# driskai/scenario_gym

Measured on AMD Instinct MI355X. Metric: entity-steps/sec (batched rollout), higher is better.
Workload: dtype f64

## Files before the change

### scenario_gym_amd/csrc/h_handle.hip

```cpp
#include "sgym_host.hpp"

using namespace sgh;

thread_local std::string sgh::g_create_err;

int sgh::fail(sg_handle *h, int code, const char *fmt, ...)
{
    char buf[512];
    va_list ap;
    va_start(ap, fmt);
    vsnprintf(buf, sizeof buf, fmt, ap);
    va_end(ap);
    if (h) h->err = buf; else g_create_err = buf;
    return code;
}

int sgh::GrowBuf::ensure(sg_handle *h, size_t bytes, bool *grew)
{
    if (grew) *grew = false;
    if (bytes <= cap) return SG_OK;
    if (ptr) HIP_TRY(h, kind == HOST ? hipHostFree(ptr) : hipFree(ptr));
    ptr = nullptr;
    cap = 0;
    HIP_TRY(h, kind == HOST ? hipHostMalloc(&ptr, bytes, hipHostMallocDefault) : hipMalloc(&ptr, bytes));
// ... 31 lines not shown
    if (cfg->device < 0 || cfg->device >= ndev)
        return fail(nullptr, SG_ERR_INVALID, "sg_create: device %d out of range (%d devices)", cfg->device, ndev);
    hipDeviceProp_t prop;
    if (hipGetDeviceProperties(&prop, cfg->device) != hipSuccess)
        return fail(nullptr, SG_ERR_HIP, "sg_create: hipGetDeviceProperties failed");
    if (strncmp(prop.gcnArchName, "gfx950", 6) != 0)
        return fail(nullptr, SG_ERR_NO_DEVICE, "sg_create: device %d is %s; this library is built for gfx950 only",
                    cfg->device, prop.gcnArchName);
    sg_handle *h = new sg_handle();
    h->cfg = *cfg;
    h->R = cfg->n_scenarios;
    h->E = cfg->n_entities;
    int G = 4;
    while (G < h->E && G < 64) G <<= 1;
    h->G = G;
    h->WV = h->E <= 64 ? 1 : (h->E <= 128 ? 2 : (h->E <= 256 ? 4 : (h->E <= 512 ? 8 : (h->E + 63) / 64)));
    h->wide = h->WV > 8;
    if (h->wide && h->R > 65535) {
        delete h;
        return fail(nullptr, SG_ERR_INVALID, "sg_create: more than 65535 scenarios of more than 512 entities in one handle (n_scenarios=%d)", cfg->n_scenarios);
    }
    h->EP = G * h->WV;
    h->sf = sg_social_force{1.5, 1.0, 1.0, 0.0, 0.5, 1.0, std::cos(200.0 / 2 * M_PI / 180), 1.3, 0.0, 0.0, 2.0, 0.1};
    h->NE = (((size_t)h->R * h->EP + 63) / 64) * 64;
    h->tab_min = env_int("SG_TAB_MIN_STEPS", h->tab_min);
    h->chunk_steps = env_int("SG_CHUNK_STEPS", h->chunk_steps);
    h->overlap = env_int("SG_OVERLAP", h->overlap);
    h->ctl_slice = std::max(1, env_int("SG_CTL_SLICE", h->ctl_slice));
    h->ped_serial = env_int("SG_PED_SERIAL", 0) != 0;
    h->crowd_kernel = env_int("SG_CROWD_KERNEL", 1);
    h->crowd_models = env_int("SG_CROWD_MODELS", 1) != 0;
    h->slice_mode = env_int("SG_SLICE", 1);
    h->queue_mode = env_int("SG_QUEUE", 1);
    h->quiet = env_int("SG_QUIET", 1) != 0;
    h->snap_d2d = env_int("SG_SNAP_D2D", 0);
    int prio_lo = 0, prio_hi = 0;
    if (hipSetDevice(cfg->device) != hipSuccess || hipStreamCreate(&h->stream) != hipSuccess ||
        hipDeviceGetStreamPriorityRange(&prio_lo, &prio_hi) != hipSuccess ||
        hipStreamCreateWithPriority(&h->ctl_stream, hipStreamNonBlocking * 0, env_int("SG_CTL_PRIO", 1) ? prio_hi : prio_lo) != hipSuccess ||
        hipEventCreate(&h->ev0) != hipSuccess || hipEventCreate(&h->ev1) != hipSuccess) {
        delete h;
        return fail(nullptr, SG_ERR_HIP, "sg_create: stream/event creation failed");
    }
    {
        int cus = 0;
        if (hipDeviceGetAttribute(&cus, hipDeviceAttributeMultiprocessorCount, cfg->device) == hipSuccess && cus > 0) h->n_simd = 4 * cus;
        else (void)hipGetLastError();
    }
    *out = h;
    return SG_OK;
}

extern "C" int sg_destroy(sg_handle *h)
{
    if (!h) return SG_OK;
    (void)hipSetDevice(h->cfg.device);
    if (h->stream) (void)hipStreamSynchronize(h->stream);
#ifdef SG_RSS_STATS
    {
        unsigned long long c[8];
        (void)hipMemcpyFromSymbol(c, HIP_SYMBOL(sg::sg_rss_stats), sizeof c);
        fprintf(stderr, "rss stats: flushes %llu groups %llu items %llu passes %llu wave-updates %llu lat-lanes %llu long-lanes %llu\n", c[0], c[1], c[2], c[3], c[4], c[5], c[6]);
    }
#endif
#ifdef SG_PHASE_TIMERS
    if (h->p.phase_cycles) {
        unsigned long long c[16];
// ... 223 lines not shown
```

### scenario_gym_amd/csrc/sgym_collide.hpp

```cpp
#pragma once

namespace sg {

struct TileCentre {
    float fs, fc;
    float fx, fy;
    float mag;
    float reach, thr;
    float nthr;
    int ix, iy;
    bool far_out;
};

__device__ __forceinline__ TileCentre tile_centre(bool present, const double *pose, double bcx, double bcy, float rad_thr,
                                                  float nbr_thr, float cell_inv)
{
    TileCentre C;
    const double x = pose[0], y = pose[1];
    sg_sincos_f32(pose[3], C.fs, C.fc);
    const float bcxf = (float)bcx, bcyf = (float)bcy;
    const float nanf_ = __builtin_nanf("");
    C.fx = present ? (float)x + (bcxf * C.fc - bcyf * C.fs) : nanf_;
    C.fy = present ? (float)y + (bcxf * C.fs + bcyf * C.fc) : nanf_;
    C.mag = __builtin_fabsf(C.fx) + __builtin_fabsf(C.fy);
    C.reach = rad_thr + 1.9073486e-6f * C.mag;
    C.thr = C.reach * C.reach;
    const float nreach = nbr_thr + 1.9073486e-6f * C.mag;
    C.nthr = nreach * nreach;
    const float ax = C.fx * cell_inv, ay = C.fy * cell_inv;
    C.ix = present ? (int)__builtin_floorf(ax) : 0;
    C.iy = present ? (int)__builtin_floorf(ay) : 0;
    C.far_out = present && !(__builtin_fabsf(ax) < 4000.0f && __builtin_fabsf(ay) < 4000.0f);
    return C;
}

template <int G>
__device__ __forceinline__ bool ego_near(const TileCentre &C, bool present, bool is_ego, int ego_lane)
{
    float ex, ey, et;
    if (G == 64) {
        ex = __int_as_float(__builtin_amdgcn_readlane(__float_as_int(C.fx), ego_lane));
        ey = __int_as_float(__builtin_amdgcn_readlane(__float_as_int(C.fy), ego_lane));
        et = __int_as_float(__builtin_amdgcn_readlane(__float_as_int(C.thr), ego_lane));
    } else {
        ex = __shfl(C.fx, ego_lane, 64);
        ey = __shfl(C.fy, ego_lane, 64);
        et = __shfl(C.thr, ego_lane, 64);
    }
    const float dx = C.fx - ex, dy = C.fy - ey;
    const float d2 = __builtin_fmaf(dy, dy, dx * dx);
    return present && !is_ego && d2 <= et;
}

template <int G, int WV, bool PED, bool CROWD = false, bool REFINE = false, typename LDS>
__device__ __forceinline__ void tile_collisions_from(const TileCentre &C, bool present, const double *pose, double velx, double vely,
                                                double dtn ,
                                                double bcx, double bcy, float trig_eps,
                                                bool is_ped_type, int sl, int tile0, LDS &L,
                                                uint64_t (&rows_out)[WV], uint64_t (&mult_rows)[WV],
                                                uint64_t (&nbr_out)[WV], bool &dense , bool *crowd_ok = nullptr,
                                                PhaseTimers *ptp = nullptr, bool hetero = false, float rmax_t = 0.0f)
{
#ifdef SG_PHASE_TIMERS
    PhaseTimers ptm_dummy;
    PhaseTimers &ptm = ptp ? *ptp : ptm_dummy;
#endif
    constexpr int TS = G * WV;
    const int slot = sl - tile0;
    const double x = pose[0], y = pose[1];
    const float fs = C.fs, fc = C.fc, fx = C.fx, fy = C.fy, mag = C.mag, reach = C.reach, thr = C.thr, nthr = C.nthr;
    const int ix = C.ix, iy = C.iy;
    const bool far_out = C.far_out;
    PH(8); tile_sync<WV>(); PH(11);
    L.cx[sl] = fx;
    L.cy[sl] = fy;
    L.cen[sl] = make_float2(fx, fy);
    L.sc[sl] = make_float2(fs, fc);
    reinterpret_cast<unsigned long long *>(L.xtab)[sl] = 0ull;
    reinterpret_cast<unsigned long long *>(L.ytab)[sl] = 0ull;
    bool insane = false;
    if (PED) {
        L.px[sl] = (!CROWD || (present && is_ped_type)) ? x : __builtin_nan("");
        L.py[sl] = y; L.vx[sl] = velx; L.vy[sl] = vely;
        L.isped[sl] = present && is_ped_type;
        const double vmag = sg_norm2(velx, vely) + 0.0000000001;
        const double uox = velx / vmag, uoy = vely / vmag, stp = vmag * dtn;
        L.ox[sl] = uox;
        L.oy[sl] = uoy;
        L.stp[sl] = stp;
        if (CROWD) {
            const double sx = stp * uox, sy = stp * uoy;
            L.sx[sl] = sx;
            L.sy[sl] = sy;
            L.ss[sl] = stp * stp;
// ... 205 lines not shown
                    const int j = tile0 + w * 64 + jl;
                    const float2 oc = L.cen[j], os = L.sc[j], oh = L.half[j];
                    float dx = oc.x - fx, dy = oc.y - fy;
                    float cd = __builtin_fabsf(__builtin_fmaf(fc, os.y, fs * os.x));
                    float sd = __builtin_fabsf(__builtin_fmaf(fs, os.y, -(fc * os.x)));
                    float g0 = __builtin_fabsf(__builtin_fmaf(dx, fc, dy * fs)) - __builtin_fmaf(oh.y, sd, __builtin_fmaf(oh.x, cd, hl));
                    float g1 = __builtin_fabsf(__builtin_fmaf(dy, fc, -(dx * fs))) - __builtin_fmaf(oh.y, cd, __builtin_fmaf(oh.x, sd, hw));
                    float g2 = __builtin_fabsf(__builtin_fmaf(dx, os.y, dy * os.x)) - __builtin_fmaf(hw, sd, __builtin_fmaf(hl, cd, oh.x));
                    float g3 = __builtin_fabsf(__builtin_fmaf(dy, os.y, -(dx * os.x))) - __builtin_fmaf(hw, cd, __builtin_fmaf(hl, sd, oh.y));
                    float gap = __builtin_fmaxf(__builtin_fmaxf(g0, g1), __builtin_fmaxf(g2, g3));
                    float eps = __builtin_fmaf(1.9073486e-6f, __builtin_fabsf(oc.x) + __builtin_fabsf(oc.y), eps_own);
                    bool unsure = (gap <= eps) && (gap >= -eps);
                    unsure = unsure || (dx == 0.0f && dy == 0.0f);
                    if (unsure) fuzzy[w] |= 1ull << jl;
                    else if (gap < -eps) rows_out[w] |= 1ull << jl;
                }
            }
            any_fuzzy = any_fuzzy || fuzzy[w] != 0;
        }
    }
#pragma unroll
    for (int w = 0; w < WV; ++w) mult_rows[w] = rows_out[w];
    PH(3);
    const bool any_fuzzy_wg = block_vote<WV>(L, 1, any_fuzzy) != 0;
    PH(15);
    if (!any_fuzzy_wg) return;

    double A[8];
    {
        double s, c;
        const double *Kp = SG_TRIG;
        asm volatile("" : "+s"(Kp));
        sg_sincos(pose[3], s, c, (ConstTbl)Kp);
        sg_corners(x, y, s, c, L.boxwl[0][sl], L.boxwl[1][sl], bcx, bcy, A);
    }
    if (WV > 1) {
#pragma unroll
        for (int k = 0; k < 8; ++k) L.cor[k][sl] = A[k];
        tile_sync<WV>();
    }
    uint64_t eq[WV];
    bool any_eq = false;
#pragma unroll
    for (int w = 0; w < WV; ++w) {
        eq[w] = 0;
        while (sg_any(fuzzy[w] != 0)) {
            const bool act = fuzzy[w] != 0;
            const int jl = act ? __builtin_ctzll(fuzzy[w]) : (slot & 63);
            if (act) fuzzy[w] &= fuzzy[w] - 1;
            const int j = tile0 + w * 64 + jl;
            double B[8];
            bool same = true;
#pragma unroll
            for (int k = 0; k < 8; ++k) {
                B[k] = WV > 1 ? L.cor[k][j] : shfl_d(A[k], j);
                same = same && (B[k] == A[k]);
            }
            if (act) {
                if (same) eq[w] |= 1ull << jl;
                else if (sg_quads_intersect(A, B)) rows_out[w] |= 1ull << jl;
            }
        }
        any_eq = any_eq || eq[w] != 0;
        mult_rows[w] = rows_out[w];
    }
    if (block_vote<WV>(L, 2, any_eq)) {
// ... 41 lines not shown
```

### scenario_gym_amd/csrc/sgym_host.hpp

```cpp
#pragma once
#include <hip/hip_runtime.h>

#include <algorithm>
#include <functional>
#include <atomic>
#include <cassert>
#include <cmath>
#include <cstdarg>
#include <cstdio>
#include <cstdlib>
#include <chrono>
#include <cstring>
#include <iterator>
#include <memory>
#include <string>
#include <thread>
#include <vector>

#include "sgym_launch.hpp"

using sg::Params;

namespace sgh {

// ... 7 lines not shown
struct GrowBuf {
    enum Kind { DEVICE, DEVICE_POISONED, HOST };
    explicit GrowBuf(Kind k) : kind(k) {}
    void *ptr = nullptr;
    size_t cap = 0;
    const Kind kind;
    int ensure(sg_handle *h, size_t bytes, bool *grew = nullptr);
    void release();
    template <typename T> T *as() const { return static_cast<T *>(ptr); }
};

struct EntityList {
    GrowBuf buf{GrowBuf::DEVICE};
    int64_t n = 0;
    int32_t *scenarios() const { return buf.as<int32_t>(); }
    int32_t *slots() const { return buf.as<int32_t>() + buf.cap / (2 * sizeof(int32_t)); }
    int upload(sg_handle *h, int64_t n_new, const int32_t *scenario, const int32_t *slot);
    void release() { buf.release(); }
};

}

struct sg_handle {
    sg_config cfg{};
    int R = 0, E = 0, EP = 0, G = 0, WV = 1;
    size_t NE = 0;
    bool wide = false;
    hipStream_t stream = nullptr;
    hipStream_t ctl_stream = nullptr;
    hipEvent_t ev0 = nullptr, ev1 = nullptr;
    int n_simd = 1024;
    int tab_min = 16, chunk_steps = 1024, overlap = 1;
    int slice_mode = 1;
    bool quiet = true;
    int queue_mode = 1;
    int ctl_slice = 64;
    int ped_serial = 0;
    int crowd_kernel = 1;
    bool crowd_models = true, models_all_sf = true;
    double c_tol = 0.4;
    uint64_t generation = 0, tick_gen = ~0ull;
    std::string err;

    bool uploaded = false;
    bool has_ped = false;
    bool planar = false;
    bool sliceable = false;
    bool all_ped = false;
    bool crowd_riders = false;
    bool ego_first = true;
    Params p{};
    sgh::ReusePool static_allocs, state_allocs;
    int32_t *d_row_scen = nullptr;
    int64_t total_rows = 0;
    std::vector<hipEvent_t> up_ev;
    std::vector<double> up_grid_t;
    sgh::GrowBuf up_stat{sgh::GrowBuf::HOST};
    std::vector<int32_t> up_row_scen;
    std::vector<std::vector<double>> up_grids;
    int n_ctl = 0;
    int n_ext = 0;
    double *d_ext = nullptr;
    int max_ctl_per_block = 0;
    std::vector<double> clock_t0;
    std::vector<int> clock_of;
    std::vector<uint8_t> slot_empty;
    unsigned char *d_reset_mask = nullptr;
// ... 389 lines not shown
```

### scenario_gym_amd/csrc/sgym_rollout.hpp

```cpp
#pragma once

namespace sg {

enum : unsigned {
    V_PED = 1,
    V_TAB = 2,
    V_HAST = 4,
    V_ROAD = 8,
    V_RSS = 16,
    V_CROWD = 32,
    V_SLICE = 64,
    V_PLANAR = 128,
    V_RIDERS = 256,
    V_CTAB = 512,
    V_MODELS = 1024
};

template <int G, int WV, unsigned F>
struct Variant {
    static constexpr bool PED = (F & V_PED) != 0, TAB = (F & V_TAB) != 0, HAST = (F & V_HAST) != 0, ROAD = (F & V_ROAD) != 0,
                          RSSV = (F & V_RSS) != 0, CROWD = (F & V_CROWD) != 0, SLICE = (F & V_SLICE) != 0, PLANAR = (F & V_PLANAR) != 0,
                          RIDERS = (F & V_RIDERS) != 0, CTAB = (F & V_CTAB) != 0, MODELS = !CROWD || (F & V_MODELS) != 0;
    static_assert(F < 2 * V_MODELS, "flags: V_* bits only");
    static_assert(!SLICE || (TAB && WV == 1 && !PED && !ROAD && !RSSV), "slices: the table variant, one wavefront per tile");
// ... 16 lines not shown
                                            const LanePtr &st)
{
    Table T;
    if (kind == SG_KIND_REPLAY) {
        size_t go = (size_t)ss.grid_off;
        T.x = p.grid_t + go; T.xs = 1;
        T.y = p.grid_y + go * 6 * p.EP + slot; T.ys = 6 * p.EP; T.cs = p.EP;
        T.n = ss.grid_n;
    } else if (kind >= SG_KIND_AGENT_REPLAY) {
        const double *kn = p.knots + fld<int64_t>(st, ST_KNOT_OFF) * 7;
        T.x = kn; T.xs = 7; T.y = kn + 1; T.ys = 7; T.cs = 1;
        T.n = (int)(fld<int64_t>(st, ST_META) >> 32);
    } else {
        T.x = nullptr; T.y = nullptr; T.n = 0; T.xs = T.ys = T.cs = 0;
    }
    return T;
}

struct SliceArgs {
    int mode;
    int n_slices, len;
    int n_total;
    const double *tt;
    const int *clock_of;
    double *dnorm;
    double2 *espeed;
    int *first_done;
    sg_event *ev;
    int *nev;
    const int *n_final;
    int slice0;
};

template <int G, int WV, unsigned F>
__device__ __forceinline__ void rollout_body_l(
    typename Variant<G, WV, F>::Lds &lds ,
    const Params &p, double timestep, int n_steps, int do_reset, int force, const double *actions ,
    const double *tab , const SliceArgs &sa = SliceArgs{},
    const unsigned bx_arg = ~0u )
{
    const unsigned bx = bx_arg == ~0u ? blockIdx.x : bx_arg;
    using V = Variant<G, WV, F>;
    constexpr bool PED = V::PED, TAB = V::TAB, ROAD = V::ROAD, RSSV = V::RSSV, CROWD = V::CROWD, SLICE = V::SLICE, PLANAR = V::PLANAR,
                   RIDERS = V::RIDERS, CTAB = V::CTAB, MODELS = V::MODELS;
    constexpr bool HAS_TAB = V::HAS_TAB, REFINE = V::REFINE, LATE = V::LATE, PARK = V::PARK;
    constexpr int NS = V::NS, TL = V::TL;
    const int tid = threadIdx.x, lane = tid & 63, wave = tid >> 6;
    const uint32_t voff = lane * 8u;
    const size_t blk = (size_t)bx * WV + wave;
    const double *st_blk = p.stat + blk * (ST_COUNT * 64);
    const LanePtr st(st_blk, voff);
    const LanePtr dy(p.dyn + blk * ((size_t)(SG_F_COLL + WV) * 64), voff);
    const int gl = bx * NS + tid;
    const int r_raw = WV == 1 ? gl / G : bx;
    const int slot = WV == 1 ? (gl & (G - 1)) : tid;
    const int tile0 = WV == 1 ? (lane & ~(G - 1)) : 0;
    const int sl = tid;
    const bool in_range = r_raw < p.R;
    const uint32_t r = in_range ? r_raw : p.R - 1;
    const ScenStatic &ss = p.sstat[r];
    sg_scenario_state &sd = p.sdyn[r];
    const int64_t meta = fld<int64_t>(st, ST_META);
    const int kind = (in_range && slot < p.E) ? (int)(meta & 0xff) : SG_KIND_NONE;
    const bool is_ped_type = ((meta >> 8) & 0xff) == 1;
    const bool is_ego = in_range && slot == ss.ego;
    const double bcx = fld(st, ST_BCX), bcy = fld(st, ST_BCY);
    const double min_t = fld(st, ST_MIN_T), max_t = fld(st, ST_MAX_T);
    const double length = ss.length;
    const bool is_static = (int)(meta >> 32) == 1;
    const bool is_agent = kind >= SG_KIND_AGENT_REPLAY;
    const bool is_replay = kind == SG_KIND_REPLAY;
    const bool replay_always = p.persist || is_static;
    float rad_thr, trig_eps, nbr_thr = 0.0f;
    float rmax_tile = 0.0f;
    bool hetero = false;
    {
        const double bw = fld(st, ST_BW), bl = fld(st, ST_BL);
        float rad = (float)(0.5 * __builtin_sqrt(bl * bl + bw * bw)) * 1.000001f;
        float off = (float)__builtin_sqrt(bcx * bcx + bcy * bcy) * 1.000001f;
        float rmax = rad, omax = off, omax_ped = (PED && is_ped_type) ? off : 0.0f;
#pragma unroll
        for (int o = 1; o < G; o <<= 1) {
            rmax = __builtin_fmaxf(rmax, __shfl_xor(rmax, o, 64));
            omax = __builtin_fmaxf(omax, __shfl_xor(omax, o, 64));
            if (PED) omax_ped = __builtin_fmaxf(omax_ped, __shfl_xor(omax_ped, o, 64));
        }
        if (WV > 1) {
            float *red = reinterpret_cast<float *>(lds.cor);
            if (lane == 0) { red[wave] = rmax; red[8 + wave] = omax; red[16 + wave] = omax_ped; }
            __syncthreads();
            for (int w = 0; w < WV; ++w) {
                rmax = __builtin_fmaxf(rmax, red[w]); omax = __builtin_fmaxf(omax, red[8 + w]);
                omax_ped = __builtin_fmaxf(omax_ped, red[16 + w]);
            }
            __syncthreads();
        }
        rad_thr = rad + rmax + 2e-3f + 2.0f * SG_TRIG32_ERR * (off + omax);
        trig_eps = SG_TRIG32_ERR * (12.0f * rad_thr + 4.0f * (off + omax));
        if (REFINE) {
// ... 41 lines not shown
                }
            }
            if (tid == 0) { lds.road_info[0] = n_staged; lds.road_info[1] = net; lds.road_info[2] = (int)net_flags; }
        }
    }
    bool crowd_static_ok = false, crowd_geom_ok = false;
    CrowdConsts CC{};
    if (CROWD) {
        const double rr = fld(st, ST_CTRL + SG_C_PED_RADIUS), hr = fld(st, ST_CTRL + SG_C_PED_HEAD_ROT);
        crowd_geom_ok = sg_all(kind != SG_KIND_AGENT_PEDESTRIAN || (hr == 0.0 && rr > 0.0 && rr < 0x1p20)) && !p.ped_serial;
        crowd_static_ok = crowd_geom_ok && crowd_params_ok(p.sf);
        const RecipDiv rs(p.sf.ped_repulse_sigma);
        CC.k2_scale = p.sf.ped_repulse_V / p.sf.ped_repulse_sigma;
        CC.sig_b = rs.b;
        CC.sig_r = rs.r;
        CC.cos_sight = p.sf.cos_sight;
        CC.sight_weight = p.sf.sight_weight;
        CC.k3 = 2 * p.sf.ped_attract_C;
    }
    bool crowd_ok = false;
    float cell_inv;
    {
        float tmax = __builtin_fmaxf(rad_thr, nbr_thr);
#pragma unroll
        for (int o = 1; o < G; o <<= 1) tmax = __builtin_fmaxf(tmax, __shfl_xor(tmax, o, 64));
        if (WV > 1) {
            float *red = reinterpret_cast<float *>(lds.cor);
            if (lane == 0) red[wave] = tmax;
            __syncthreads();
            for (int w = 0; w < WV; ++w) tmax = __builtin_fmaxf(tmax, red[w]);
            __syncthreads();
        }
        cell_inv = 1.0f / (1.05f * tmax + 0.05f);
    }
    const double *wp = nullptr;
    int nwp = 0;
    if (PED && kind == SG_KIND_AGENT_PEDESTRIAN) {
        int64_t rt = fld<int64_t>(st, ST_ROUTE);
        wp = p.routes + (rt & 0xffffffffffffll) * 2;
        nwp = (int)(rt >> 48);
    }

    double pose[6], dist, t, prev_t;
    double velx = 0.0, vely = 0.0;
    CtrlState cs;
    double m_avg, m_max, m_t;
    uint64_t last_row[WV];
    long long noise_pos = 0;
    int n_ev, goal_idx = 0;
    bool present;
    int done, steps;
    uint64_t row[WV], mult_rows[WV], nbr[WV];
    bool dense = false;
    const int64_t ctl_q = HAS_TAB ? fld<int64_t>(st, ST_CTL) : -1;
    const bool tab_lane = HAS_TAB && ctl_q >= 0 && (kind == SG_KIND_AGENT_PID || kind == SG_KIND_AGENT_VEHICLE);
    const size_t tab_lane_stride = (size_t)(p.tab_steps + 1) * CT_W;
    const bool rider = (RIDERS && kind != SG_KIND_NONE && kind != SG_KIND_AGENT_PEDESTRIAN) ||
                       (CTAB && (kind == SG_KIND_AGENT_PID || kind == SG_KIND_AGENT_VEHICLE));
    const double *rider_row = (RIDERS || CTAB) ? tab + (size_t)(rider ? fld<int64_t>(st, ST_CTL) : 0) * tab_lane_stride : nullptr;
    int last_k = -1;
    int cl[TL];
    const double *cb[TL];
    double sx[TL], sy[TL], sh[TL];
    if (HAS_TAB) {
        uint64_t cm = __ballot(tab_lane);
#pragma unroll
// ... 265 lines not shown
        Table T = lane_table(p, kind, ss, slot, st);
        S.cur = seg_locate(T, t);
        seg_load(T, S);
    }

    if (HAS_TAB && n_steps > 0) tab_issue(true);

    int k = 0;
    bool all_done = false;
    bool vel_clean_prev = false;
    const bool vel_every_step = !LATE || (p.term_mask & ~SG_TERM_MAX_LENGTH) != 0 || sg_any(is_ego && !tab_lane);
    auto rows_again = [](const LanePtr &o) {
        LanePtr q = o;
        if (LATE) {
            asm volatile("" : "+v"(q.a[0]));
            q.a[1] = q.a[0] + 8 * ROW;
            q.a[2] = q.a[0] + 16 * ROW;
        }
        return q;
    };
    auto dy_again = [&]() {
        if (!LATE) return dy;
        uint32_t voff_o = voff;
        asm volatile("" : "+v"(voff_o));
        return LanePtr(p.dyn + blk * ((size_t)(SG_F_COLL + WV) * 64), voff_o);
    };
    auto sd_again = [&]() -> sg_scenario_state & {
        if (!LATE) return sd;
        uint32_t r_o = r;
        asm volatile("" : "+v"(r_o));
        return p.sdyn[r_o];
    };
    const bool quiet_on = V::QUIET && p.quiet != 0 && (p.term_mask & ~SG_TERM_MAX_LENGTH) == 0 && p.rec_cap == 0;
    PhaseTimers ptm;
#ifdef SG_PHASE_TIMERS
    ptm.start();
    if (lane == 0 && bx < 1024) p.phase_cycles[16 + bx * 4 + wave] = __builtin_amdgcn_s_getreg((4 << 0) | (0 << 6) | (31 << 11));
#endif
    sg_loads_done();
    sg_lgkm_done();
    while (k < n_steps && !all_done) {
    if (!CROWD && t + timestep > S.x_hi) {
        int kind_o = kind, slot_o = slot;
        LanePtr st_o = st;
        asm volatile("" : "+v"(kind_o), "+v"(slot_o), "+v"(st_o.a[0]));
        Table T = lane_table(p, kind_o, ss, slot_o, st_o);
        seg_advance(T, S, t + timestep);
        sg_loads_done();
    }
    for (; k < n_steps; ++k) {
        if (!CROWD && sg_any(t + timestep > S.x_hi)) break;
        const bool warm = SLICE && k == 0;
        const bool run_lane = in_range && (force || !done) && !(SLICE && k == 0 && slice_a == 0);
        PH(5);
        const bool any_run_ = WV == 1 ? sg_any(run_lane || (SLICE && k == 0 && in_range && !done)) : run_lane;
        PH(7);
        if (!any_run_) { all_done = true; break; }
        const bool run = (G == 64 && WV == 1 && !SLICE) ? true : run_lane;
        const double *Kp = SG_TRIG;
        if (!TAB) asm volatile("" : "+s"(Kp));
        ConstTbl K = (ConstTbl)Kp;

        const double next_t = t + timestep;
        const double state_dt = t - prev_t;
        const double dt = next_t - t;
        double act_a = 0.0, act_s = 0.0;
// ... 218 lines not shown
            RecipDiv rd(dt);
            if (PLANAR) {
                flat = !SLICE && sg_all(dt > 0.0);
            } else {
                const uint32_t zbits = (uint32_t)(__double2hiint(d[2]) | __double2hiint(d[4]) | __double2hiint(d[5])) |
                                       (uint32_t)(__double2loint(d[2]) | __double2loint(d[4]) | __double2loint(d[5]));
                flat = !SLICE && sg_all((!run | !npres | (present & (zbits == 0))) & (dt > 0.0));
            }
            auto lo_ok = [](double a) { return (__builtin_fabs(a) >= 0x1p-959) | (__double_as_longlong(a) == 0); };
            double dmax = __builtin_fmax(__builtin_fmax(__builtin_fabs(d[0]), __builtin_fabs(d[1])), __builtin_fabs(d[3]));
            bool safe = rd.ok & lo_ok(d[0]) & lo_ok(d[1]) & lo_ok(d[3]);
            if (!flat) {
                dmax = __builtin_fmax(__builtin_fmax(dmax, __builtin_fabs(d[2])), __builtin_fmax(__builtin_fabs(d[4]), __builtin_fabs(d[5])));
                safe = safe & lo_ok(d[2]) & lo_ok(d[4]) & lo_ok(d[5]);
            }
            safe = safe & (dmax < 0x1p961);
            if (sg_all(safe)) {
                vel[0] = rd.div(d[0]); vel[1] = rd.div(d[1]); vel[3] = rd.div(d[3]);
                if (flat) {
                    vel[2] = vel[4] = vel[5] = 0.0;
                } else {
                    vel[2] = rd.div(d[2]); vel[4] = rd.div(d[4]); vel[5] = rd.div(d[5]);
                }
            } else {
#pragma unroll
                for (int c = 0; c < 6; ++c) vel[c] = d[c] / dt;
            }
        }

        const bool vel_zpr_clean = vel_clean_prev;
        vel_clean_prev = flat;
        const bool was_present = present;
        if (run) {
            present = npres;
            if (npres) {
                if (PLANAR) {
                    pose[0] = np_[0]; pose[1] = np_[1]; pose[3] = np_[3];
                } else {
#pragma unroll
                    for (int c = 0; c < 6; ++c) pose[c] = np_[c];
                }
                if (!SLICE) dist += PLANAR ? sg_norm2(d[0], d[1])  : sg_norm3(d[0], d[1], d[2]);
                if (PED) { velx = vel[0]; vely = vel[1]; }
            }
            prev_t = t;
            t = next_t;
            ++steps;
            last_k = k;
            if (SLICE && sa.mode == 0 && !warm) {
                sa.dnorm[((size_t)blk * (size_t)(sa.n_total + 1) + (size_t)steps) * 64 + lane] = npres ? sg_norm3(d[0], d[1], d[2]) : 0.0;
                if (is_ego)
                    sa.espeed[(size_t)steps * p.R + r] =
                        make_double2(present ? sg_norm3(vel[0], vel[1], vel[2]) : __builtin_nan(""),
                                     (was_present && steps > 1) ? 1.0 - prev_t / t : __builtin_nan(""));
            }
            if (LATE) {
                if (need_vel && present) {
                    const LanePtr dv = dy_again();
#pragma unroll
                    for (int c = 0; c < 6; ++c) stf(dv, SG_F_VEL + c, vel[c]);
                }
            } else if (!SLICE || (sa.mode == 1 && !warm)) {
            stf(dy, SG_F_POSE + 0, pose[0]); stf(dy, SG_F_POSE + 1, pose[1]); stf(dy, SG_F_POSE + 3, pose[3]);
            if (!flat) { stf(dy, SG_F_POSE + 2, pose[2]); stf(dy, SG_F_POSE + 4, pose[4]); stf(dy, SG_F_POSE + 5, pose[5]); }
            if (present) {
                stf(dy, SG_F_VEL + 0, vel[0]); stf(dy, SG_F_VEL + 1, vel[1]); stf(dy, SG_F_VEL + 3, vel[3]);
                if (!(flat && vel_zpr_clean)) {
                    stf(dy, SG_F_VEL + 2, vel[2]); stf(dy, SG_F_VEL + 4, vel[4]); stf(dy, SG_F_VEL + 5, vel[5]);
                }
            }
            stf(dy, SG_F_DIST, dist);
            if (SLICE || sg_any(present != was_present)) stf(dy, SG_F_PRESENT, (uint64_t)present);
            }
            if (PED && kind == SG_KIND_AGENT_PEDESTRIAN) {
                stf(dy, SG_F_FORCE + 0, fpx);
                stf(dy, SG_F_FORCE + 1, fpy);
            }
            if (p.rec_cap > 0 && steps < p.rec_cap) {
                int nan_hi = 0x7ff80000;
                if (!CROWD) asm volatile("" : "+s"(nan_hi));
                const double absent = __hiloint2double(nan_hi, 0);
#pragma unroll
                for (int c = 0; c < 6; ++c)
                    p.rec_pose[((size_t)steps * 6 + c) * p.R * p.EP + (size_t)r * p.EP + slot] = present ? pose[c] : absent;
                if (slot == 0) { p.rec_t[(size_t)steps * p.R + r] = t; sd_again().rec_rows = steps + 1; }
            }
            if (!SLICE && is_ego && present && !tab_lane) {
                if (CROWD) { m_avg = lds.ego_m[0]; m_max = lds.ego_m[1]; m_t = lds.ego_m[2]; }
                if (PARK) ego_fetch();
                double speed = sg_norm3(vel[0], vel[1], vel[2]);
                double w = m_t / t;
                m_avg += (1.0 - w) * (speed - m_avg);
                m_t = t;
                m_max = __builtin_fmax(speed, m_max);
                if (CROWD) { lds.ego_m[0] = m_avg; lds.ego_m[1] = m_max; lds.ego_m[2] = m_t; }
                if (PARK) ego_park();
            }
        }
        PH(1);
        const TileCentre cen = tile_centre(present, pose, bcx, bcy, rad_thr, nbr_thr, cell_inv);
        bool quiet = false;
        if (V::QUIET && quiet_on && k != n_steps - 1) {
            const bool ends = (p.term_mask & SG_TERM_MAX_LENGTH) && (t + dt > length);
            const uint64_t ego_mask = __ballot(is_ego);
            int ego_lane = (int)__builtin_ctzll(ego_mask | (1ull << 63));
            if (G < 64) {
                const uint32_t half = lane < 32 ? (uint32_t)ego_mask : (uint32_t)(ego_mask >> 32);
                ego_lane = tile0 + (int)(__builtin_ctz((half >> (tile0 & 31)) | 0x80000000u) & (G - 1));
            }
            quiet = !sg_any(run_lane & (ends | ego_near<G>(cen, present, is_ego, ego_lane)));
        }
        if (V::QUIET && quiet) {
            if (run && is_ego) row[0] = 0;
        } else {
            uint64_t nrow[WV];
            tile_collisions_from<G, WV, PED, CROWD, REFINE>(cen, present, pose, velx, vely, (t + timestep) - t, bcx, bcy, trig_eps,
                                                            is_ped_type, sl, tile0, lds, nrow, mult_rows, nbr, dense, &crowd_ok, &ptm, hetero, rmax_tile);
            if (run) {
#pragma unroll
                for (int w = 0; w < WV; ++w) {
                    const bool row_moved = !LATE && (SLICE || sg_any(nrow[w] != row[w]));
                    row[w] = nrow[w];
                    if ((!SLICE || (sa.mode == 1 && !warm)) && row_moved) stf(dy, SG_F_COLL + w, row[w]);
                }
            }
        }

        int ndone = 0;
        if ((p.term_mask & SG_TERM_MAX_LENGTH) && (t + dt > length)) ndone = 1;
        if (p.term_mask & (SG_TERM_COLLISION | SG_TERM_EGO_COLLISION)) {
            bool any_mine = false;
#pragma unroll
            for (int w = 0; w < WV; ++w) any_mine = any_mine || row[w] != 0;
            bool any_tile, ego0;
            if (WV == 1) {
                uint64_t m = __ballot(any_mine) >> tile0;
                if (G < 64) m &= (1ull << (G & 63)) - 1;
                any_tile = m != 0;
                uint64_t row0 = __shfl(row[0], tile0, 64);
                ego0 = ((__ballot(present) >> tile0) & 1) && row0 != 0;
            } else {
                any_tile = __syncthreads_or(any_mine);
                ego0 = __syncthreads_or(tid == 0 && present && any_mine);
            }
            if ((p.term_mask & SG_TERM_COLLISION) && any_tile) ndone = 1;
            if ((p.term_mask & SG_TERM_EGO_COLLISION) && ego0) ndone = 1;
        }
        if (ROAD && (p.term_mask & SG_TERM_EGO_OFF_ROAD)) {
            bool off = false;
            if (sl == tile0 && in_range) {
// ... 147 lines not shown
        } else if ((RIDERS || CTAB) && rider) {
            if (last_k >= 0 && (kind == SG_KIND_AGENT_PID || kind == SG_KIND_AGENT_VEHICLE)) {
                const double *lr = rider_row + (size_t)last_k * CT_W;
                const double *lr1 = lr + (size_t)p.n_ctl_pad * tab_lane_stride;
                stf(dx, SG_F_CTRL + 0, lr[CT_SPEED]); stf(dx, SG_F_CTRL + 1, lr1[CT_ELON]);
                stf(dx, SG_F_CTRL + 2, lr1[CT_ELAT]); stf(dx, SG_F_CTRL + 3, lr1[CT_EINT]);
            }
        } else {
            stf(dx, SG_F_CTRL + 0, cs.speed); stf(dx, SG_F_CTRL + 1, cs.e_lon_prev);
            stf(dx, SG_F_CTRL + 2, cs.e_lat_prev); stf(dx, SG_F_CTRL + 3, cs.e_lon_int);
        }
        if (slot == 0) { sx.t = t; sx.prev_t = prev_t; sx.done = done; sx.n_steps = steps; if (PED) sx.noise_pos = noise_pos; }
        if (RSSV) {
            if (slot < p.E) {
                p.rss_state[rss_idx] = rss_st;
                if (rss_touched) {
                    p.rss_code[rss_idx] = rss_cd;
                    p.rss_safe[(size_t)rss_idx * 2] = rss_lat;
                    p.rss_safe[(size_t)rss_idx * 2 + 1] = rss_long;
                }
            }
            if (slot == 0 && rss_touched) p.rss_seen[r] = steps;
        }
        if (is_ego) {
            sx.ego_avg_speed = m_avg; sx.ego_max_speed = m_max; sx.avg_t = m_t;
            if (steps > 0 && present) sx.ego_distance_travelled = dist;
#pragma unroll
            for (int w = 0; w < WV; ++w) (w < 4 ? sx.last_row[w & 3] : sx.last_row_hi[w & 3]) = last_row[w];
            sx.n_events = n_ev;
        }
    }
}

template <int G, int WV, unsigned F>
__device__ __forceinline__ void rollout_body(
    const Params &p, double timestep, int n_steps, int do_reset, int force, const double *actions, const double *tab,
    const SliceArgs &sa = SliceArgs{}, const unsigned bx_arg = ~0u)
{
    __shared__ typename Variant<G, WV, F>::Lds lds;
    rollout_body_l<G, WV, F>(lds, p, timestep, n_steps, do_reset, force, actions, tab, sa, bx_arg);
}

struct TabGroups {
    unsigned long long active, bufof[2];
    int gsz, n[4];
    const double *buf[4];
    unsigned start0, len0, start1, len1;
    __device__ __forceinline__ unsigned map(unsigned i) const { return i < len0 ? start0 + i : start1 + (i - len0); }
    __device__ __forceinline__ bool pick(unsigned blk, int &n_steps, const double *&tab) const
    {
        const unsigned g = blk / (unsigned)gsz;
        if (!((active >> g) & 1)) return false;
        const unsigned b = (unsigned)(bufof[g >> 5] >> (2 * (g & 31))) & 3u;
        n_steps = b == 0 ? n[0] : (b == 1 ? n[1] : (b == 2 ? n[2] : n[3]));
        tab = b == 0 ? buf[0] : (b == 1 ? buf[1] : (b == 2 ? buf[2] : buf[3]));
        return true;
    }
};

template <int G, int WV, bool PED, bool TAB>
__global__ __launch_bounds__(64 * WV, PED ? SG_WAVES_PER_SIMD_PED : (TAB ? SG_WAVES_PER_SIMD_TAB : SG_WAVES_PER_SIMD)) void rollout_kernel(
    Params p, double timestep, int n_steps, int do_reset, int force, const double *actions, const double *tab)
{
    constexpr unsigned F = (PED ? V_PED : 0u) | (TAB ? V_TAB : 0u) | (TAB && WV > 1 ? V_HAST : 0u);
    rollout_body<G, WV, F>(p, timestep, n_steps, do_reset, force, actions, tab);
}

template <int WV>
__global__ __launch_bounds__(64 * WV, SG_WAVES_PER_SIMD_PED) void rollout_kernel_crowd(
    Params p, double timestep, int n_steps, int do_reset, int force, const double *actions, const double *tab)
{
    rollout_body<64, WV, V_PED | V_CROWD>(p, timestep, n_steps, do_reset, force, actions, tab);
}
// ... 32 lines not shown
{
    int n_steps;
    const double *tab;
    const unsigned blk = tg.map(blockIdx.x);
    if (!tg.pick(blk, n_steps, tab)) return;
    rollout_body<G, 1, V_RSS | V_CTAB>(p, timestep, n_steps, 0, force, nullptr, tab, SliceArgs{}, blk);
}

template <int G, int WV>
__global__ __launch_bounds__(64 * WV, SG_WAVES_PER_SIMD) void rollout_kernel_rss_road(
    Params p, double timestep, int n_steps, int do_reset, int force, const double *actions, const double *tab)
{
    rollout_body<G, WV, V_ROAD | V_RSS>(p, timestep, n_steps, do_reset, force, actions, tab);
}
template <int G, int WV>
__global__ __launch_bounds__(64 * WV, SG_WAVES_PER_SIMD_PED) void rollout_kernel_rss_ped(
    Params p, double timestep, int n_steps, int do_reset, int force, const double *actions, const double *tab)
{
    rollout_body<G, WV, V_PED | V_RSS>(p, timestep, n_steps, do_reset, force, actions, tab);
}

#ifndef SG_TAB_WAVES
#define SG_TAB_WAVES 3
#define SG_TAB_VGPR 84
#endif
template <int G>
__global__ __launch_bounds__(64, SG_TAB_WAVES) __attribute__((amdgpu_num_vgpr(SG_TAB_VGPR))) void rollout_kernel_tab(
    Params p, double timestep, int force, TabGroups tg)
{
    int n_steps;
    const double *tab;
    const unsigned blk = tg.map(blockIdx.x);
    if (!tg.pick(blk, n_steps, tab)) return;
    rollout_body<G, 1, V_TAB | V_HAST>(p, timestep, n_steps, 0, force, nullptr, tab, SliceArgs{}, blk);
}
#ifndef SG_PLANAR_WAVES
#define SG_PLANAR_WAVES 3
#define SG_PLANAR_VGPR 84
#endif
template <int G>
__global__ __launch_bounds__(64, SG_PLANAR_WAVES) __attribute__((amdgpu_num_vgpr(SG_PLANAR_VGPR))) void rollout_kernel_tab_planar(
    Params p, double timestep, int force, TabGroups tg)
{
    int n_steps;
    const double *tab;
    const unsigned blk = tg.map(blockIdx.x);
    if (!tg.pick(blk, n_steps, tab)) return;
    rollout_body<G, 1, V_TAB | V_HAST | V_PLANAR>(p, timestep, n_steps, 0, force, nullptr, tab, SliceArgs{}, blk);
}

template <int G>
__global__ __launch_bounds__(64, SG_WAVES_PER_SIMD_TAB) void rollout_kernel_slice(Params p, double timestep, SliceArgs sa)
{
    rollout_body<G, 1, V_TAB | V_SLICE>(p, timestep, 0, 0, 0, nullptr, nullptr, sa);
}
template <int G>
__global__ __launch_bounds__(64, SG_WAVES_PER_SIMD_TAB) void rollout_kernel_slice_tab(Params p, double timestep, SliceArgs sa, const double *tab)
{
    rollout_body<G, 1, V_TAB | V_HAST | V_SLICE>(p, timestep, 0, 0, 0, nullptr, tab, sa);
}

#ifdef SG_UNIT_MAIN
static __global__ __launch_bounds__(64) void clock_kernel(const double *t0 , int n_clocks, double timestep, int n_total, double *tt)
{
    const int c = blockIdx.x * 64 + threadIdx.x;
    if (c >= n_clocks) return;
    double *row = tt + (size_t)c * (size_t)(n_total + 1);
    double t = t0[c];
    row[0] = t;
    int j = 1;
    for (; j + 15 <= n_total; j += 16) {
        double v[16];
#pragma unroll
        for (int u = 0; u < 16; ++u) { t = t + timestep; v[u] = t; }
#pragma unroll
        for (int u = 0; u < 16; ++u) row[j + u] = v[u];
    }
    for (; j <= n_total; ++j) { t = t + timestep; row[j] = t; }
}
#endif

// ... 127 lines not shown
```

Baseline: 148.8 billion.

## Add conservative ego-distance slack to skip quiet-step proximity checks

```diff
diff --git a/scenario_gym_amd/csrc/h_handle.hip b/scenario_gym_amd/csrc/h_handle.hip
--- a/scenario_gym_amd/csrc/h_handle.hip
+++ b/scenario_gym_amd/csrc/h_handle.hip
@@ -87,7 +87,7 @@
     h->crowd_models = env_int("SG_CROWD_MODELS", 1) != 0;
     h->slice_mode = env_int("SG_SLICE", 1);
     h->queue_mode = env_int("SG_QUEUE", 1);
-    h->quiet = env_int("SG_QUIET", 1) != 0;
+    { const int q = env_int("SG_QUIET", 1); h->quiet = q == 0 ? 0 : q == 2 ? 2 : 1; }
     h->snap_d2d = env_int("SG_SNAP_D2D", 0);
     int prio_lo = 0, prio_hi = 0;
     if (hipSetDevice(cfg->device) != hipSuccess || hipStreamCreate(&h->stream) != hipSuccess ||
diff --git a/scenario_gym_amd/csrc/sgym_collide.hpp b/scenario_gym_amd/csrc/sgym_collide.hpp
--- a/scenario_gym_amd/csrc/sgym_collide.hpp
+++ b/scenario_gym_amd/csrc/sgym_collide.hpp
@@ -12,13 +12,12 @@
     bool far_out;
 };
 
-__device__ __forceinline__ TileCentre tile_centre(bool present, const double *pose, double bcx, double bcy, float rad_thr,
+__device__ __forceinline__ TileCentre tile_centre(bool present, const double *pose, float bcxf, float bcyf, float rad_thr,
                                                   float nbr_thr, float cell_inv)
 {
     TileCentre C;
     const double x = pose[0], y = pose[1];
     sg_sincos_f32(pose[3], C.fs, C.fc);
-    const float bcxf = (float)bcx, bcyf = (float)bcy;
     const float nanf_ = __builtin_nanf("");
     C.fx = present ? (float)x + (bcxf * C.fc - bcyf * C.fs) : nanf_;
     C.fy = present ? (float)y + (bcxf * C.fs + bcyf * C.fc) : nanf_;
@@ -33,9 +32,14 @@
     C.far_out = present && !(__builtin_fabsf(ax) < 4000.0f && __builtin_fabsf(ay) < 4000.0f);
     return C;
 }
+__device__ __forceinline__ TileCentre tile_centre(bool present, const double *pose, double bcx, double bcy, float rad_thr,
+                                                  float nbr_thr, float cell_inv)
+{
+    return tile_centre(present, pose, (float)bcx, (float)bcy, rad_thr, nbr_thr, cell_inv);
+}
 
 template <int G>
-__device__ __forceinline__ bool ego_near(const TileCentre &C, bool present, bool is_ego, int ego_lane)
+__device__ __forceinline__ bool ego_near(const TileCentre &C, bool present, bool is_ego, int ego_lane, float *d2_out = nullptr)
 {
     float ex, ey, et;
     if (G == 64) {
@@ -49,7 +53,56 @@
     }
     const float dx = C.fx - ex, dy = C.fy - ey;
     const float d2 = __builtin_fmaf(dy, dy, dx * dx);
+    if (d2_out) *d2_out = d2;
     return present && !is_ego && d2 <= et;
+}
+
+#define SG_SLACK_EPS 1.0e-5f
+#define SG_SLACK_DELTA 0x1p-15f
+#define SG_SLACK_CAP 256.0f
+#define SG_SLACK_MAG 65536.0f
+
+template <int G>
+__device__ __forceinline__ float ego_bcast(float v, int ego_lane)
+{
+    if (G == 64) return __int_as_float(__builtin_amdgcn_readlane(__float_as_int(v), ego_lane));
+    return __shfl(v, ego_lane, 64);
+}
+
+__device__ __forceinline__ float ego_turn(float bcxf, float bcyf)
+{
+    return (__builtin_fabsf(bcxf) + __builtin_fabsf(bcyf)) * 1.000001f;
+}
+
+__device__ __forceinline__ float ego_move(double step_len, double dh, float bcxf, float bcyf)
+{
+    const float dhf = __builtin_fabsf((float)dh);
+    return __builtin_fmaf(__builtin_fabsf(bcxf), dhf, __builtin_fmaf(__builtin_fabsf(bcyf), dhf, (float)step_len));
+}
+
+template <int G>
+__device__ __forceinline__ float ego_slack_step(float slack, float mv, bool appears, int lane, int ego_lane)
+{
+    const float mv_ego = ego_bcast<G>(mv, ego_lane);
+    slack = __builtin_fmaf(-(1.0f + SG_SLACK_EPS), (mv + mv_ego) + SG_SLACK_DELTA, slack);
+    const uint64_t app = __ballot(appears);
+    if (app) {
+        const uint64_t mine = (1ull << lane) | (1ull << ego_lane);
+        if (app & mine) slack = 0.0f;
+    }
+    return slack;
+}
+
+template <int G>
+__device__ __forceinline__ float ego_slack_refresh(const TileCentre &C, float d2, float off, bool present, int ego_lane)
+{
+    const float er = ego_bcast<G>(C.reach, ego_lane), em = ego_bcast<G>(C.mag, ego_lane), eo = ego_bcast<G>(off, ego_lane);
+    const float D = __builtin_sqrtf(d2);
+    const float margin = __builtin_fmaf(0x1p-19f, D + er, __builtin_fmaf(3.6e-7f, C.mag + em, 4.0e-5f * (off + eo)));
+    const float s = (D - er) - margin;
+    const bool small = (C.mag < SG_SLACK_MAG) & (em < SG_SLACK_MAG);
+    const float kept = small ? (s < SG_SLACK_CAP ? s : SG_SLACK_CAP) : 0.0f;
+    return (!present | (em != em)) ? SG_SLACK_CAP : kept;
 }
 
 template <int G, int WV, bool PED, bool CROWD = false, bool REFINE = false, typename LDS>
@@ -59,7 +112,8 @@
                                                 bool is_ped_type, int sl, int tile0, LDS &L,
                                                 uint64_t (&rows_out)[WV], uint64_t (&mult_rows)[WV],
                                                 uint64_t (&nbr_out)[WV], bool &dense , bool *crowd_ok = nullptr,
-                                                PhaseTimers *ptp = nullptr, bool hetero = false, float rmax_t = 0.0f)
+                                                PhaseTimers *ptp = nullptr, bool hetero = false, float rmax_t = 0.0f,
+                                                const LanePtr *bc_row = nullptr )
 {
 #ifdef SG_PHASE_TIMERS
     PhaseTimers ptm_dummy;
@@ -331,6 +385,11 @@
         const double *Kp = SG_TRIG;
         asm volatile("" : "+s"(Kp));
         sg_sincos(pose[3], s, c, (ConstTbl)Kp);
+        if (bc_row) {
+            bcx = fld(*bc_row, ST_BCX);
+            bcy = fld(*bc_row, ST_BCY);
+            sg_loads_done();
+        }
         sg_corners(x, y, s, c, L.boxwl[0][sl], L.boxwl[1][sl], bcx, bcy, A);
     }
     if (WV > 1) {
diff --git a/scenario_gym_amd/csrc/sgym_host.hpp b/scenario_gym_amd/csrc/sgym_host.hpp
--- a/scenario_gym_amd/csrc/sgym_host.hpp
+++ b/scenario_gym_amd/csrc/sgym_host.hpp
@@ -63,7 +63,7 @@
     int n_simd = 1024;
     int tab_min = 16, chunk_steps = 1024, overlap = 1;
     int slice_mode = 1;
-    bool quiet = true;
+    int quiet = 1;
     int queue_mode = 1;
     int ctl_slice = 64;
     int ped_serial = 0;
diff --git a/scenario_gym_amd/csrc/sgym_rollout.hpp b/scenario_gym_amd/csrc/sgym_rollout.hpp
--- a/scenario_gym_amd/csrc/sgym_rollout.hpp
+++ b/scenario_gym_amd/csrc/sgym_rollout.hpp
@@ -72,7 +72,7 @@
     int slice0;
 };
 
-template <int G, int WV, unsigned F>
+template <int G, int WV, unsigned F, bool SLACK = true>
 __device__ __forceinline__ void rollout_body_l(
     typename Variant<G, WV, F>::Lds &lds ,
     const Params &p, double timestep, int n_steps, int do_reset, int force, const double *actions ,
@@ -105,6 +105,7 @@
     const bool is_ped_type = ((meta >> 8) & 0xff) == 1;
     const bool is_ego = in_range && slot == ss.ego;
     const double bcx = fld(st, ST_BCX), bcy = fld(st, ST_BCY);
+    const float bcxf = (float)bcx, bcyf = (float)bcy;
     const double min_t = fld(st, ST_MIN_T), max_t = fld(st, ST_MAX_T);
     const double length = ss.length;
     const bool is_static = (int)(meta >> 32) == 1;
@@ -212,6 +213,7 @@
             __syncthreads();
         }
         cell_inv = 1.0f / (1.05f * tmax + 0.05f);
+        if (V::QUIET && G == 64) cell_inv = __int_as_float(__builtin_amdgcn_readfirstlane(__float_as_int(cell_inv)));
     }
     const double *wp = nullptr;
     int nwp = 0;
@@ -543,6 +545,17 @@
         return p.sdyn[r_o];
     };
     const bool quiet_on = V::QUIET && p.quiet != 0 && (p.term_mask & ~SG_TERM_MAX_LENGTH) == 0 && p.rec_cap == 0;
+    const bool slack_on = SLACK && quiet_on && p.quiet == 2;
+    float slack = 0.0f;
+    auto ego_lane_of = [&]() {
+        const uint64_t ego_mask = __ballot(is_ego);
+        int ego_lane = (int)__builtin_ctzll(ego_mask | (1ull << 63));
+        if (G < 64) {
+            const uint32_t half = lane < 32 ? (uint32_t)ego_mask : (uint32_t)(ego_mask >> 32);
+            ego_lane = tile0 + (int)(__builtin_ctz((half >> (tile0 & 31)) | 0x80000000u) & (G - 1));
+        }
+        return ego_lane;
+    };
     PhaseTimers ptm;
 #ifdef SG_PHASE_TIMERS
     ptm.start();
@@ -827,6 +840,7 @@
         vel_clean_prev = flat;
         const bool was_present = present;
         if (run) {
+            float mv = 0.0f;
             present = npres;
             if (npres) {
                 if (PLANAR) {
@@ -835,9 +849,14 @@
 #pragma unroll
                     for (int c = 0; c < 6; ++c) pose[c] = np_[c];
                 }
-                if (!SLICE) dist += PLANAR ? sg_norm2(d[0], d[1])  : sg_norm3(d[0], d[1], d[2]);
+                if (!SLICE) {
+                    const double step_len = PLANAR ? sg_norm2(d[0], d[1])  : sg_norm3(d[0], d[1], d[2]);
+                    dist += step_len;
+                    if (V::QUIET && slack_on) mv = ego_move(step_len, d[3], bcxf, bcyf);
+                }
                 if (PED) { velx = vel[0]; vely = vel[1]; }
             }
+            if (V::QUIET && slack_on) slack = ego_slack_step<G>(slack, mv, present & !was_present, lane, ego_lane_of());
             prev_t = t;
             t = next_t;
             ++steps;
@@ -893,24 +912,33 @@
             }
         }
         PH(1);
-        const TileCentre cen = tile_centre(present, pose, bcx, bcy, rad_thr, nbr_thr, cell_inv);
+        const bool eligible = V::QUIET && quiet_on && k != n_steps - 1;
         bool quiet = false;
-        if (V::QUIET && quiet_on && k != n_steps - 1) {
-            const bool ends = (p.term_mask & SG_TERM_MAX_LENGTH) && (t + dt > length);
-            const uint64_t ego_mask = __ballot(is_ego);
-            int ego_lane = (int)__builtin_ctzll(ego_mask | (1ull << 63));
-            if (G < 64) {
-                const uint32_t half = lane < 32 ? (uint32_t)ego_mask : (uint32_t)(ego_mask >> 32);
-                ego_lane = tile0 + (int)(__builtin_ctz((half >> (tile0 & 31)) | 0x80000000u) & (G - 1));
-            }
-            quiet = !sg_any(run_lane & (ends | ego_near<G>(cen, present, is_ego, ego_lane)));
+        bool ends = false;
+        if (V::QUIET && eligible) {
+            ends = (p.term_mask & SG_TERM_MAX_LENGTH) && (t + dt > length);
+            if (slack_on) quiet = !sg_any(run_lane & (ends | (present & !is_ego & !(slack > 0.0f))));
+        }
+        TileCentre cen;
+        if (!(V::QUIET && quiet)) {
+            cen = V::QUIET ? tile_centre(present, pose, bcxf, bcyf, rad_thr, nbr_thr, cell_inv)
+                           : tile_centre(present, pose, bcx, bcy, rad_thr, nbr_thr, cell_inv);
+            if (V::QUIET && eligible) {
+                const int ego_lane = ego_lane_of();
+                float d2;
+                quiet = !sg_any(run_lane & (ends | ego_near<G>(cen, present, is_ego, ego_lane, &d2)));
+                if (slack_on) slack = ego_slack_refresh<G>(cen, d2, ego_turn(bcxf, bcyf), present, ego_lane);
+            }
         }
         if (V::QUIET && quiet) {
             if (run && is_ego) row[0] = 0;
         } else {
             uint64_t nrow[WV];
-            tile_collisions_from<G, WV, PED, CROWD, REFINE>(cen, present, pose, velx, vely, (t + timestep) - t, bcx, bcy, trig_eps,
-                                                            is_ped_type, sl, tile0, lds, nrow, mult_rows, nbr, dense, &crowd_ok, &ptm, hetero, rmax_tile);
+            LanePtr st_o = st;
+            if (V::QUIET) asm volatile("" : "+v"(st_o.a[0]));
+            tile_collisions_from<G, WV, PED, CROWD, REFINE>(cen, present, pose, velx, vely, (t + timestep) - t, V::QUIET ? 0.0 : bcx,
+                                                            V::QUIET ? 0.0 : bcy, trig_eps, is_ped_type, sl, tile0, lds, nrow, mult_rows, nbr,
+                                                            dense, &crowd_ok, &ptm, hetero, rmax_tile, V::QUIET ? &st_o : nullptr);
             if (run) {
 #pragma unroll
                 for (int w = 0; w < WV; ++w) {
@@ -1124,13 +1152,13 @@
     }
 }
 
-template <int G, int WV, unsigned F>
+template <int G, int WV, unsigned F, bool SLACK = true>
 __device__ __forceinline__ void rollout_body(
     const Params &p, double timestep, int n_steps, int do_reset, int force, const double *actions, const double *tab,
     const SliceArgs &sa = SliceArgs{}, const unsigned bx_arg = ~0u)
 {
     __shared__ typename Variant<G, WV, F>::Lds lds;
-    rollout_body_l<G, WV, F>(lds, p, timestep, n_steps, do_reset, force, actions, tab, sa, bx_arg);
+    rollout_body_l<G, WV, F, SLACK>(lds, p, timestep, n_steps, do_reset, force, actions, tab, sa, bx_arg);
 }
 
 struct TabGroups {
@@ -1229,7 +1257,7 @@
     const double *tab;
     const unsigned blk = tg.map(blockIdx.x);
     if (!tg.pick(blk, n_steps, tab)) return;
-    rollout_body<G, 1, V_TAB | V_HAST>(p, timestep, n_steps, 0, force, nullptr, tab, SliceArgs{}, blk);
+    rollout_body<G, 1, V_TAB | V_HAST, false>(p, timestep, n_steps, 0, force, nullptr, tab, SliceArgs{}, blk);
 }
 #ifndef SG_PLANAR_WAVES
 #define SG_PLANAR_WAVES 3
@@ -1243,7 +1271,7 @@
     const double *tab;
     const unsigned blk = tg.map(blockIdx.x);
     if (!tg.pick(blk, n_steps, tab)) return;
-    rollout_body<G, 1, V_TAB | V_HAST | V_PLANAR>(p, timestep, n_steps, 0, force, nullptr, tab, SliceArgs{}, blk);
+    rollout_body<G, 1, V_TAB | V_HAST | V_PLANAR, false>(p, timestep, n_steps, 0, force, nullptr, tab, SliceArgs{}, blk);
 }
 
 template <int G>
```

Measured after the change: 134.7 billion. 9.5% lower.
